# zitongbai/bipedal_control

Measured on AMD Instinct MI355X. Metric: MPC solves/s (H1, horizon=100), higher is better.
Workload: dtype f64; 1 GPU; Unitree H1 trot (template tiled from t = 0), horizon=100 intervals (dt 0.015), batch=256 per GPU perturbed initial states, cold start, 1 SQP iteration (BASELINE.json configs[1]); solver=sqp, global_batch=256, problems_on_rank0=256, shooting_nodes=108, nx=22, nu=22

## Files before the change

bipedal_control_amd/csrc/kernels/riccati_fast.h:

```cpp
#pragma once
#include <hip/hip_runtime.h>

#include "../device_model.h"
#include "riccati.h"
#include "project_node.h"
#include "linesearch.h"

namespace bpmpc {

struct RiccatiFastIO {
  RiccatiIO base;
  const double *Wt, *Qp, *Mt;
  const double* Vt;
  const double *lqA, *lqB, *lqb, *lqq, *lqr, *qrd, *gdt;
  const DeviceModel* model;
  const double* zero_one;
  const int* mode;
  double *Acl, *bcl;
  double *kff;
  double *mvec, *mscal;
  double* Kfull;
  double* prof;
  int k_lo, k_hi;
  double* carry;
  double reg;
  bool with_ls;
  ProblemLS ls;
};

__device__ __forceinline__ void lds_barrier() {
  __builtin_amdgcn_fence(__ATOMIC_RELEASE, "workgroup", "local");
  __builtin_amdgcn_s_barrier();
  __builtin_amdgcn_fence(__ATOMIC_ACQUIRE, "workgroup", "local");
}
__device__ __forceinline__ void lds_wave_sync() {
  __builtin_amdgcn_fence(__ATOMIC_RELEASE, "wavefront", "local");
  __builtin_amdgcn_wave_barrier();
  __builtin_amdgcn_fence(__ATOMIC_ACQUIRE, "wavefront", "local");
}
__device__ __forceinline__ double readlane_f64(double v, int lane) {
  const int lo = __builtin_amdgcn_readlane(__double2loint(v), lane);
  const int hi = __builtin_amdgcn_readlane(__double2hiint(v), lane);
  return __hiloint2double(hi, lo);
}
template <int NJ>
__device__ __forceinline__ void linesearch_begin_wave(double* partial , const ProblemLS& p, int lane) {
  constexpr int NX = 12 + NJ;
  {
    double a = 0.0, b = 0.0, c = 0.0;
    for (int k = lane; k < p.n_nodes; k += kWave) { a += p.node_perf[3 * k]; b += p.node_perf[3 * k + 1]; c += p.node_perf[3 * k + 2]; }
    if (lane < NX) { const double d = p.x0[lane] - p.x[lane]; b += d * d; }
    partial[lane] = a; partial[kWave + lane] = b; partial[2 * kWave + lane] = c;
  }
  lds_wave_sync();
  if (lane < 3) {
    double s = 0.0;
    for (int i = 0; i < kWave; ++i) s += partial[lane * kWave + i];
// ... 336 lines not shown
```

bipedal_control_amd/csrc/kernels/riccati_mfma.h:

```cpp
#pragma once
#include <hip/hip_runtime.h>

#include "riccati_fast.h"


namespace bpmpc {

typedef double v4d __attribute__((ext_vector_type(4)));

template <int LD>
struct LdsRows {
  static constexpr int kCols = LD;
  __host__ __device__ static constexpr int ix(int row, int col) { return row * LD + col; }
  static constexpr int size(int rows) { return rows * LD; }
};
template <int NBC>
struct LdsSwz {
  static constexpr int kCols = 16 * NBC, PS = 32 * NBC + 2;
  __host__ __device__ static constexpr int ix(int row, int col) { return (row >> 1) * PS + ((col >> 4) << 5) + (((row ^ (col >> 4)) & 1) << 4) + (col & 15); }
  static constexpr int size(int rows) { return ((rows + 1) / 2) * PS; }
};

template <int NJ>
struct RiccatiMfmaWorkspace {
// ... 142 lines not shown
        jix[e] = (ok && col == row) ? 1.0 : 0.0; jiy[e] = (ok && col + 1 == row) ? 1.0 : 0.0;
        jbo[e] = (ok && col == NX) ? row : -1; jb[e] = 0.0;
      }
    }
#pragma unroll
    for (int e = 0; e < SW; ++e) { const int p = tp + e * NLD; const bool ok = p < NPW; wo[e] = ok ? LW::ix(p / HW, 2 * (p % HW)) : -1; wc[e] = 2 * (p % HW); }
#pragma unroll
    for (int e = 0; e < SQ; ++e) { const int p = tp + e * NLD; const bool ok = p < NPQ; qo[e] = ok ? LN::ix(p / HQU, 2 * (p % HQU)) : -1; }
#pragma unroll
    for (int e = 0; e < SM; ++e) { const int p = tp + e * NLD; const bool ok = p < NPM; mo[e] = ok ? LW::ix(p / HW, 2 * (p % HW)) : -1; mc[e] = 2 * (p % HW); mr[e] = p / HW; }
  }
  __device__ __forceinline__ void prefetch(int nt, int mode) {
    const int cend = 16 * ((BC + nt + 15) >> 4);
#pragma unroll
    for (int e = 0; e < SW; ++e) {
      if constexpr (AM) { if ((e + 1) * NLD <= NPW || wo[e] >= 0) { const double2 v = *(wc[e] < cend ? gW + e * NLD : reinterpret_cast<const double2*>(pw.zero_one + 2)); wx[e] = v.x; wy[e] = v.y; } }
      else if (((e + 1) * NLD <= NPW || wo[e] >= 0) && wc[e] < cend) { const double2 v = gW[e * NLD]; wx[e] = v.x; wy[e] = v.y; }
    }
#pragma unroll
    for (int e = 0; e < SQ; ++e) if ((e + 1) * NLD <= NPQ || qo[e] >= 0) { const int p = tl + e * NLD; const double2 v = gQ[(p / HQU) * HQ + p % HQU]; qx[e] = v.x; qy[e] = v.y; }
#pragma unroll
    for (int e = 0; e < SM; ++e) {
      if constexpr (AM) { if ((e + 1) * NLD <= NPM || mo[e] >= 0) { const double2 v = *((mr[e] < nt && mc[e] < cend) ? gM + e * NLD : reinterpret_cast<const double2*>(pw.zero_one + 2)); mx[e] = v.x; my[e] = v.y; } }
      else if (((e + 1) * NLD <= NPM || mo[e] >= 0) && mr[e] < nt && mc[e] < cend) { const double2 v = gM[e * NLD]; mx[e] = v.x; my[e] = v.y; }
    }
    pw.prefetch(nt, mode);
    if constexpr (JR) {
      dtk = *gDt;
#pragma unroll
      for (int e = 0; e < SVJ; ++e) jb[e] = *(jbo[e] >= 0 ? gB + jbo[e] : pw.zero_one);
      gB -= NX; gDt -= 1;
    }
    gW -= PL::W_SIZE / 2; gQ -= PL::Q_SIZE / 2; gM -= PL::M_SIZE / 2;
  }
  __device__ __forceinline__ void stage(double* W, double* PW, double* Qq, double* M, double* rvec, int nt) const {
    stage_wm(W, M, rvec, nt);
    stage_pq(PW, Qq);
  }
  __device__ __forceinline__ void stage_wm(double* Wf, double* Mf, double* rvec, int nt) const {
    const int cend = 16 * ((BC + nt + 15) >> 4);
#pragma unroll
    for (int e = 0; e < SW; ++e)
      if ((e + 1) * NLD <= NPW || wo[e] >= 0) {
        const bool in = AM || wc[e] < cend; double2 v; v.x = in ? wx[e] : 0.0; v.y = in ? wy[e] : 0.0; *reinterpret_cast<double2*>(Wf + wo[e]) = v;
      }
#pragma unroll
    for (int e = 0; e < SM; ++e)
      if ((e + 1) * NLD <= NPM || mo[e] >= 0) {
        const bool in = AM || (mr[e] < nt && mc[e] < cend);
        double2 v; v.x = in ? mx[e] : 0.0; v.y = in ? my[e] : 0.0;
        *reinterpret_cast<double2*>(Mf + mo[e]) = v;
        if (mc[e] == NX) rvec[mr[e]] = v.x;
      }
    if constexpr (JR) {
#pragma unroll
      for (int e = 0; e < SVJ; ++e)
        if ((e + 1) * NLD <= NJ * HW || pw.vo[e] >= 0) {
          double2 v; v.x = __builtin_fma(dtk, pw.vx[e], jix[e] + jb[e]); v.y = __builtin_fma(dtk, pw.vy[e], jiy[e]);
          *reinterpret_cast<double2*>(Wf + pw.vo[e]) = v;
        }
    }
  }
  __device__ __forceinline__ void stage_pq(double* PW, double* Qf) const {
#pragma unroll
    for (int e = 0; e < SQ; ++e)
      if ((e + 1) * NLD <= NPQ || qo[e] >= 0) { double2 v; v.x = qx[e]; v.y = qy[e]; *reinterpret_cast<double2*>(Qf + qo[e]) = v; }
// ... 714 lines not shown
```

bipedal_control_amd/csrc/kernels/riccati_mfma8.h:

```cpp
#pragma once
#include <hip/hip_runtime.h>

#include "riccati_mfma.h"

namespace bpmpc {

typedef unsigned int bp8_u32x2 __attribute__((ext_vector_type(2)));
constexpr int kRiccati8Threads = 512;

template <int NJ>
struct RiccatiMfma8Workspace {
  static constexpr int NX = 12 + NJ, NU = 12 + NJ;
  static constexpr int RB = 32;
  static constexpr int RE = 16;
  static constexpr int WC = NX + 1 + NU;
  using LN = LdsSwz<2>;
  using LW = LdsSwz<(WC + 15) / 16>;
  static constexpr int ZN = 31;
  static_assert(NX + 1 <= 32 && NU <= 32, "two block rows / columns");
  alignas(16) double S[LN::size(RB)];
  alignas(16) double Qq[2][LN::size(RB)];
  alignas(16) double Sn[LN::size(RB)];
  alignas(16) double Zt[LN::size(RE)];
  alignas(16) double Yn[LN::size(RE)];
  alignas(16) double W[2][LW::size(RB)];
  alignas(16) double PW[2][LW::size(RB)];
  alignas(16) double SW[LW::size(RB)];
  alignas(16) double M[2][LW::size(RE)];
  alignas(16) double Mb[LW::size(RE)];
  double r[2][NU];
  int status;
  unsigned char nut[kMaxRiccatiStages];
  unsigned char mode[kMaxRiccatiStages];
};
template <class L>
__device__ __forceinline__ v4d sblk_load(const double* Mx, int r0, int c0, int l) {
  v4d c;
#pragma unroll
  for (int r = 0; r < 4; ++r) c[r] = lds1(Mx[L::ix(r0 + (l >> 4) + 4 * r, c0 + (l & 15))]);
  return c;
}
template <class L>
__device__ __forceinline__ void sblk_store(double* Mx, int r0, int c0, int l, v4d c) {
#pragma unroll
  for (int r = 0; r < 4; ++r) Mx[L::ix(r0 + (l >> 4) + 4 * r, c0 + (l & 15))] = c[r];
}

template <int ROWS, class Emit>
__device__ __forceinline__ bool forward_eliminate_wave(double (&v)[ROWS], int nt, Emit&& emit) {
  bool ok = true;
#pragma unroll
  for (int p = 0; p < ROWS; ++p) {
    if (p < nt) {
      double f[ROWS];
#pragma unroll
      for (int i = p; i < ROWS; ++i) f[i] = readlane_f64(v[i], p);
      ok = ok && (f[p] > 0.0);
      const double row = v[p] * fast_reciprocal(f[p]);
      emit(p, v[p], row);
#pragma unroll
      for (int i = p + 1; i < ROWS; ++i) v[i] -= f[i] * row;
      v[p] = row;
    }
  }
  return ok;
}
// ... 30 lines not shown
  const int k_top = (io.k_hi < N ? io.k_hi : N) - 1;
  const bool resumed = io.k_hi < N;
  {
    double* z = &ws.S[0];
    constexpr int total = (int)(offsetof(WS, status) / sizeof(double));
    for (int idx = tid; idx < total; idx += NT) z[idx] = 0.0;
  }
  __syncthreads();
  if (tid == 0) ws.status = resumed ? (int)io.carry[NXX + NX] : 0;
  if (!resumed && io.reg != 0.0 && tid < NX) ws.S[LN::ix(tid, tid)] = io.reg;
  if (resumed) {
    for (int idx = tid; idx < NXX; idx += NT) ws.S[LN::ix(idx / NX, idx % NX)] = io.carry[idx];
    if (tid < NX) ws.S[LN::ix(tid, NX)] = io.carry[NXX + tid];
  }
  int too_wide = 0;
  for (int idx = tid; idx < N && idx < kMaxRiccatiStages; idx += NT) {
    const int n = io.base.nut[idx];
    ws.nut[idx] = (unsigned char)n;
    ws.mode[idx] = (unsigned char)(n > 0 ? (io.mode[idx] & 3) : kModeEvent);
    too_wide |= n > RE ? 1 : 0;
  }
  if (__syncthreads_or(too_wide)) {
    if (tid == 0) {
      if (io.k_lo > 0) io.carry[NXX + NX] = 1.0;
      else { io.base.summary[0] = 0.0; io.base.summary[1] = 0.0; io.base.summary[2] = 0.0; io.base.summary[3] = 1.0; }
    }
    if (io.k_lo == 0 && io.with_ls && tid < kWave) linesearch_begin_wave<NJ>(&ws.S[0], io.ls, tid);
    return;
  }

  constexpr int NLD = kLoaders * kWave;
  PackedStageLoader<NJ, NLD, RE, LW::kCols, LN::kCols, true, !JW, LW, LN> ld;
  ld.init(io, (w - 4) * kWave + l, role_l, (size_t)(k_top > 0 ? k_top : 0));
  if (role_l && k_top >= io.k_lo) {
    const int kt = k_top > 0 ? k_top : 0, n0 = io.base.nut[kt];
    ld.prefetch(n0, n0 > 0 ? (io.mode[kt] & 3) : kModeEvent);
  }
  __syncthreads();
#ifdef BPMPC_RICCATI_PROFILE
  long long tacc[8] = {0, 0, 0, 0, 0, 0, 0, 0};
  long long tprev = clock64();
#define RM8PROF(slot) do { const long long tn_ = clock64(); tacc[slot] += tn_ - tprev; tprev = tn_; } while (0)
#define RM8OWN(phase) do { if (BPMPC_RICCATI_PROFILE == 10 + (phase)) tacc[7] += clock64() - tprev; } while (0)
#else
#define RM8PROF(slot) ((void)0)
#define RM8OWN(phase) ((void)0)
#endif

  constexpr int PSN = LN::PS, PSW = LW::PS;
  const int hk = lk >> 1, pk = lk & 1, hl = li >> 1, pl = li & 1;
  auto opaque = [](int v) { asm volatile("" : "+v"(v)); return v; };
  const int nP2a = opaque(hk * PSN + 16 * pk + li), nP2b = opaque(hk * PSN + 16 * (pk ^ 1) + li);
  const int wP2a = opaque(hk * PSW + 16 * pk + li), wP2b = opaque(hk * PSW + 16 * (pk ^ 1) + li);
  const int nP1a = opaque(hl * PSN + 16 * pl + lk), nP1b = opaque(hl * PSN + 16 * (pl ^ 1) + lk);
  const int nSV = opaque(hk * PSN + 16 * (pk ^ 1) + 32 + (NX & 15));
  static_assert(NX >= 16 && NX < 32, "column nx lies in block column 1");
  int wBC;
  { const int c = BC + li, cb = c >> 4; wBC = opaque(hk * PSW + 32 * cb + 16 * ((pk ^ cb) & 1) + (c & 15)); }
  int foW, foY, foB[4], snN, snP, wA3, suN, suZ, suY;
  {
    const int bw = w < 3 ? w : 3, r0 = 16 * (bw >> 1), c0 = 16 * (bw & 1);
    foW = opaque((r0 / 2) * PSW + 2 * c0 + ((bw & 1) ? wP2b : wP2a));
    foY = opaque(2 * c0 + ((bw & 1) ? wP2b : wP2a));
#pragma unroll
    for (int ks = 0; ks < 4; ++ks) foB[ks] = opaque(LW::ix(r0 + li, BC + 4 * ks + lk));
    const int sid = w & 1;
    snN = opaque(32 * sid + (sid ? nP2b : nP2a));
    snP = opaque(32 * sid + (sid ? wP2b : wP2a));
    const int ac3 = 16 + li < NX ? 16 + li : NX - 1;
// ... 30 lines not shown
    for (int r = 0; r < 4; ++r) { acl[r] = lds1(W[foW + 2 * r * PSW]); kf[r] = lds1(PW[foW + 2 * r * PSW]); }
    double ab[4], ap[4], yb[4];
#pragma unroll
    for (int ks = 0; ks < 4; ++ks) {
      yb[ks] = lds1(M[foY + 2 * ks * PSW]);
      ab[ks] = lds1(W[foB[ks]]);
      ap[ks] = lds1(PW[foB[ks]]);
    }
    __builtin_amdgcn_sched_barrier(0);
#pragma unroll
    for (int ks = 0; ks < 4; ++ks) {
      if (ks < ksn) {
        acl = __builtin_amdgcn_mfma_f64_16x16x4f64(ab[ks], yb[ks], acl, 0, 0, 0);
        kf = __builtin_amdgcn_mfma_f64_16x16x4f64(ap[ks], yb[ks], kf, 0, 0, 0);
      }
    }
    const unsigned ku = (unsigned)__builtin_amdgcn_readfirstlane(k);
    const unsigned sm = ku * (unsigned)(NXX * 8), sv = ku * (unsigned)(NX * 8);
#pragma unroll
    for (int r = 0; r < 4; ++r) {
      bp8_u32x2 va, vk;
      va.x = (unsigned)__double2loint(acl[r]); va.y = (unsigned)__double2hiint(acl[r]);
      vk.x = (unsigned)__double2loint(kf[r]); vk.y = (unsigned)__double2hiint(kf[r]);
      __builtin_amdgcn_raw_buffer_store_b64(va, rAcl, oom[r], sm, 0);
      __builtin_amdgcn_raw_buffer_store_b64(vk, rKf, oom[r], sm, 0);
      if (c0 != 0) {
        __builtin_amdgcn_raw_buffer_store_b64(va, rbcl, oov[r], sv, 0);
        __builtin_amdgcn_raw_buffer_store_b64(vk, rkff, oov[r], sv, 0);
      }
    }
  };

  auto finish_m = [&](int k, int buf) {
    if (l <= NX) {
      const int fm0 = 32 * (l >> 4) + 16 * ((l >> 4) & 1) + (l & 15);
      double yv[RE], rv[RE];
#pragma unroll
      for (int i = 0; i < RE; ++i) { yv[i] = ws.M[buf][(i >> 1) * PSW + ((i & 1) ? (fm0 ^ 16) : fm0)]; rv[i] = ws.r[buf][i]; }
      double m0 = l < NX ? ws.Qq[buf][LN::ix(l, NX)] : 0.0, m1 = 0.0;
#pragma unroll
      for (int i = 0; i < RE; i += 2) { m0 += yv[i] * rv[i]; m1 += yv[i + 1] * rv[i + 1]; }
      if (l < NX) io.mvec[(size_t)k * NX + l] = m0 + m1; else io.mscal[k] = m0 + m1;
    }
  };

  int pend_k = -1, pend_nt = 0;
  for (int k = k_top; k >= io.k_lo; --k) {
    const int nt = ws.nut[k];
    const int cur = k & 1;
    double* const W = ws.W[cur];
    double* const PW = ws.PW[cur];
    double* const Qq = ws.Qq[cur];
    double* const M = ws.M[cur];
    double* const rvec = ws.r[cur];
    const int ksn = (nt + 3) >> 2;
    const int nbc = (BC + nt + 15) >> 4;
    auto sn_block = [&](auto top_c) {
      constexpr bool TOP = decltype(top_c)::value;
      const int nb = TOP ? snN : 8 * PSN + 32 + nP2b;
      const int wa = TOP ? wP2a : wA3;
      const int wb = TOP ? snP : 32 + wP2b;
      v4d acc;
#pragma unroll
      for (int r = 0; r < 4; ++r) acc[r] = lds1(Qq[nb + 2 * r * PSN]);
      double a[KS], b[KS];
#pragma unroll
      for (int ks = 0; ks < KS; ++ks) {
        a[ks] = lds1(W[wa + 2 * ks * PSW]);
        b[ks] = lds1(ws.SW[wb + 2 * ks * PSW]);
      }
      if constexpr (!TOP) {
#pragma unroll
        for (int ks = 0; ks < KS; ++ks) a[ks] *= amask3;
      }
      __builtin_amdgcn_sched_barrier(0);
#pragma unroll
      for (int ks = 0; ks < KS; ++ks) acc = __builtin_amdgcn_mfma_f64_16x16x4f64(a[ks], b[ks], acc, 0, 0, 0);
#pragma unroll
      for (int r = 0; r < 4; ++r) ws.Sn[nb + 2 * r * PSN] = acc[r];
    };
    if (role_l) ld.stage(W, PW, Qq, M, rvec, nt);
    RM8OWN(0);
    lds_barrier();
    RM8PROF(0);
    if (role_l && k > io.k_lo) ld.prefetch(ws.nut[k - 1], ws.mode[k - 1]);
    if (w != 4 && w != 5) {
      const int id = w < 4 ? w : w - 2;
      if (id < 2 * nbc) {
        const int bi = id >= nbc ? 1 : 0;
        const int r0 = 16 * bi, c0 = 16 * (id - bi * nbc);
        const int row = r0 + li;
        const double half = row < NX ? 0.5 : 0.0;
        constexpr int KG1 = KS - 4;
        const int odd = (c0 >> 4) & 1;
        const int wb = 2 * c0 + (odd ? wP2b : wP2a);
        const int sx0 = 8 * bi * PSN + nP1a, sx1 = 8 * bi * PSN + 32 + nP1b;
        const int sy = 32 * bi + (bi ? nP2b : nP2a);
        double a[KS], b[KS], sv[4], ga[4];
#pragma unroll
        for (int ks = 0; ks < KS; ++ks) {
          const bool up = (bi == 0 && ks >= 4), lo = (bi != 0 && ks < 4);
          const int ex = (ks < 4 ? sx0 : sx1) + 4 * (ks & 3), ey = sy + 2 * ks * PSN;
          a[ks] = half * (lds1(ws.S[lo ? ey : ex]) + lds1(ws.S[up ? ex : ey]));
          b[ks] = lds1(W[wb + 2 * ks * PSW]);
        }
        const double smask = (c0 + li == NX) ? 1.0 : 0.0;
#pragma unroll
        for (int r = 0; r < 4; ++r) sv[r] = smask * lds1(ws.S[nSV + (8 * bi + 2 * r) * PSN]);
#pragma unroll
        for (int ks = 0; ks < 4; ++ks) ga[ks] = (bi == 0 || ks < KG1) ? lds1(W[wBC + (8 * bi + 2 * ks) * PSW]) : 0.0;
        v4d g;
#pragma unroll
        for (int r = 0; r < 4; ++r) g[r] = lds1(M[wb + 2 * r * PSW]);
        if (bi != 0) g = v4d{0.0, 0.0, 0.0, 0.0};
        __builtin_amdgcn_sched_barrier(0);
        v4d acc = {sv[0], sv[1], sv[2], sv[3]};
#pragma unroll
        for (int ks = 0; ks < KS; ++ks) acc = __builtin_amdgcn_mfma_f64_16x16x4f64(a[ks], b[ks], acc, 0, 0, 0);
// ... 62 lines not shown
        else BP_GJ_CASE(10, (forward_eliminate_rows<10, true>), back_substitute_rows)
      } else {
        if (nt <= 12) BP_GJ_CASE(12, forward_eliminate_wave<12>, back_substitute_wave)
        else BP_GJ_CASE(RE, forward_eliminate_wave<RE>, back_substitute_wave)
      }
#undef BP_GJ_CASE
#undef BP_EM
    } else {
      if (w == 4 || w == 5) sn_block(std::true_type{});
      if (w == 4) sn_block(std::false_type{});
      if (w == 5 && pend_k >= 0) finish_m(pend_k, cur ^ 1);
      if ((w < 3 || role_f) && pend_k >= 0) finish_outputs(pend_k, cur ^ 1, pend_nt, w < 3 ? w : 3);
      RM8PROF(6);
      lds_barrier();
      RM8PROF(3);
      if (role_c && w != 2) {
        v4d acc;
#pragma unroll
        for (int r = 0; r < 4; ++r) acc[r] = lds1(ws.Sn[suN + 2 * r * PSN]);
        double ag[4], yb[4];
#pragma unroll
        for (int ks = 0; ks < 4; ++ks) {
          ag[ks] = -lds1(ws.Zt[suZ + 2 * ks * PSN]);
          yb[ks] = lds1(ws.Yn[suY + 2 * ks * PSN]);
        }
        __builtin_amdgcn_sched_barrier(0);
#pragma unroll
        for (int ks = 0; ks < 4; ++ks)
          if (ks < ksn) acc = __builtin_amdgcn_mfma_f64_16x16x4f64(ag[ks], yb[ks], acc, 0, 0, 0);
#pragma unroll
        for (int r = 0; r < 4; ++r) ws.S[suN + 2 * r * PSN] = acc[r];
      }
    }
    pend_k = k; pend_nt = nt;
    RM8OWN(4);
    RM8PROF(4);
  }
#ifdef BPMPC_RICCATI_PROFILE
#if BPMPC_RICCATI_PROFILE == 2
  if (io.prof && l == 0) io.prof[w] = (double)tacc[6];
#elif BPMPC_RICCATI_PROFILE >= 10
  if (io.prof && l == 0) io.prof[w] = (double)tacc[7];
#else
  if (io.prof && tid == 0)
    for (int i = 0; i < 5; ++i) io.prof[i] = (double)tacc[i];
  if (io.prof && tid == 7 * kWave) io.prof[7] = (double)tacc[6];
#endif
#endif
  __syncthreads();
  if ((w < 3 || role_f) && pend_k >= 0) finish_outputs(pend_k, pend_k & 1, pend_nt, w < 3 ? w : 3);
  if (w == 5 && pend_k >= 0) finish_m(pend_k, pend_k & 1);
  __syncthreads();
  if (io.k_lo > 0) {
    for (int idx = tid; idx < NXX; idx += NT) { const int r = idx / NX, c = idx % NX; io.carry[idx] = (r >= 16 && c < 16) ? ws.S[LN::ix(c, r)] : ws.S[LN::ix(r, c)]; }
    if (tid < NX) io.carry[NXX + tid] = ws.S[LN::ix(tid, NX)];
    if (tid == 0) io.carry[NXX + NX] = (double)ws.status;
    return;
  }
  {
    const int st = ws.status;
    __syncthreads();
#ifdef BPMPC_RICCATI_PROFILE
    const long long tr0 = clock64();
#endif
    constexpr int kRingChunk = 4;
    using RR = RolloutRing<NJ, NT, kRingChunk>;
    constexpr int kRingCap = RR::cap((int)(offsetof(WS, status) / sizeof(double)));
    static_assert(kRingCap >= 128, "roll-out history");
    riccati_rollout_ring<NJ, NT, kRingChunk>(reinterpret_cast<double*>(&ws), kRingCap, st, io);
#ifdef BPMPC_RICCATI_PROFILE
    if (BPMPC_RICCATI_PROFILE == 1 && io.prof && tid == 0) io.prof[5] = (double)(clock64() - tr0);
#endif
  }
}

}
```

bipedal_control_amd/csrc/launch.h:

```cpp
#pragma once
#include <hip/hip_runtime.h>

#include <cstddef>

#include "device_model.h"
#include "kernels/linesearch.h"
#include "kernels/node_lq.h"
#include "kernels/project_node.h"
#include "kernels/riccati_fast.h"
#include "kernels/linearize_fast.h"

namespace bpmpc {

struct Buffers {
  int *g_kind, *g_mode, *g_nodes;
  double *g_dt, *g_start, *g_zref, *g_zdref;
  int* p_grid;
  double *p_x0, *p_tgt_t, *p_tgt_x;
  int* p_tgt_n;
  double *x, *u, *x_init, *u_init, *xref;
  double *A, *B, *b, *Q, *R, *P, *q, *r, *c, *C, *D, *e, *perf;
  int* nc;
  double *Px, *Pu, *Pe, *At, *Bt, *bt, *Qt, *Rt, *Pt, *qt, *rt;
  double *Wt, *Qp, *Mt;
// ... 14 lines not shown
  int *rg_gait, *rg_status, *rg_rows, *lib_i;
  double* ric_carry;
  double* zero_page;
  double *trial_perf, *base, *alpha, *stats;
  int *done, *active, *iterations, *remaining;
};

struct DdpBuffers {
  int cap;
  int nv;
  double alpha_v[kMaxDdpSteps];
  double* lff;
  double *rec_t, *rec_x, *rec_u, *cost;
  int* rec_n;
  double *end_x, *end_u;
  int *roll_steps, *roll_status;
  double *sol_t, *sol_x, *sol_u;
  int* sol_n;
  double *merit0, *merit, *alpha, *update_is;
  int *accepted, *failed, *n_points;
};

constexpr int kLinMaxEvents = 8;
struct Launch {
  const DeviceModel* model;
  Buffers buf;
  int batch, N;
  int k0, klen;
  int cold;
  int feedback;
  int serial_legs;
  LineSearchSettings ls;
  double reg_prim;
  int lin_ev_n, lin_inter;
  int lin_ev[kLinMaxEvents];
  int ilqr;
  double ilqr_shift;
};


template <int NJ>
__device__ __forceinline__ NodeInputs node_inputs(const Launch& L, int b, int k) {
  constexpr int NX = 12 + NJ, NU = 12 + NJ;
  const int g = L.buf.p_grid[b];
  const size_t gs = (size_t)g * L.N + k, s = (size_t)b * L.N + k;
  NodeInputs in;
  in.kind = L.buf.g_kind[gs];
  in.mode = L.buf.g_mode[gs];
  in.dt = L.buf.g_dt[gs];
  in.x = L.buf.x + ((size_t)b * (L.N + 1) + k) * NX;
  in.xnext = in.x + NX;
  in.u = L.buf.u + s * NU;
  in.xref = L.buf.xref + s * NX;
  in.zref = L.buf.g_zref + gs * 4;
  in.zdref = L.buf.g_zdref + gs * 4;
  return in;
}

template <int NJ>
__device__ __forceinline__ NodeInputs node_inputs_on_grid(const Launch& L, int b, int k, int g) {
  constexpr int NX = 12 + NJ, NU = 12 + NJ;
  const size_t gs = (size_t)g * L.N + k, s = (size_t)b * L.N + k;
  NodeInputs in;
  in.kind = L.buf.g_kind[gs];
  in.mode = L.buf.g_mode[gs];
  in.dt = L.buf.g_dt[gs];
// ... 41 lines not shown
    if (io.with_ls && tid_ < kWave) linesearch_begin_wave<NJ>(lds_scratch, io.ls, tid_);
    return false;
  }
  const size_t s0 = (size_t)b * L.N;
  double* dx0 = L.buf.dx0 + (size_t)b * NX;
  if (tid_ < NX) dx0[tid_] = L.buf.p_x0[(size_t)b * NX + tid_] - L.buf.x[(size_t)b * (L.N + 1) * NX + tid_];
  __syncthreads();
  io.base.N = L.buf.g_nodes[L.buf.p_grid[b]];
  io.base.nut = L.buf.nut + s0;
  io.base.At = L.buf.At + s0 * NX * NX; io.base.Bt = L.buf.Bt + s0 * NX * NU; io.base.bt = L.buf.bt + s0 * NX;
  io.base.Qt = L.buf.Qt + s0 * NX * NX; io.base.Rt = L.buf.Rt + s0 * NU * NU; io.base.Pt = L.buf.Pt + s0 * NU * NX;
  io.base.qt = L.buf.qt + s0 * NX; io.base.rt = L.buf.rt + s0 * NU;
  io.Wt = L.buf.Wt + s0 * PackedLq<NJ>::W_SIZE; io.Qp = L.buf.Qp + s0 * PackedLq<NJ>::Q_SIZE; io.Mt = L.buf.Mt + s0 * PackedLq<NJ>::M_SIZE;
  io.base.Px = L.buf.Px + s0 * NU * NX; io.base.Pu = L.buf.Pu + s0 * NU * NU; io.base.Pe = L.buf.Pe + s0 * NU;
  io.Vt = L.buf.Vt + s0 * NJ * PackedLq<NJ>::WP;
  io.mode = L.buf.g_mode + (size_t)L.buf.p_grid[b] * L.N;
  io.zero_one = L.buf.zero_page;
  io.lqA = L.buf.A + s0 * NX * NX; io.lqB = L.buf.B + s0 * NX * NU; io.lqb = L.buf.b + s0 * NX; io.lqq = L.buf.q + s0 * NX; io.lqr = L.buf.r + s0 * NU;
  io.qrd = L.buf.qrd + s0 * kQrdStride; io.gdt = L.buf.g_dt + (size_t)L.buf.p_grid[b] * L.N;
  io.model = L.model;
  io.base.dx0 = dx0;
  io.base.Kt = nullptr; io.base.kt = nullptr;
  io.base.dx = L.buf.dx + (size_t)b * (L.N + 1) * NX; io.base.du = L.buf.du + s0 * NU;
  io.base.K = nullptr;
  io.base.summary = L.buf.summary + (size_t)b * 4;
  io.Acl = L.buf.Acl + s0 * NX * NX; io.bcl = L.buf.bcl + s0 * NX; io.kff = L.buf.kff + s0 * NU;
  io.mvec = L.buf.mvec + s0 * NX; io.mscal = L.buf.mscal + s0;
  io.Kfull = L.buf.K + s0 * NU * NX;
  io.prof = L.buf.rprof ? L.buf.rprof + (size_t)b * 8 : nullptr;
  io.k_lo = L.k0;
  io.k_hi = L.k0 + L.klen;
  io.carry = L.buf.ric_carry + (size_t)b * (NX * NX + NX + 2);
  io.reg = L.reg_prim;
  return true;
}

}
```

bipedal_control_amd/csrc/solver.h:

```cpp
#pragma once
#include <hip/hip_runtime.h>

#include <algorithm>
#include <cstring>
#include <map>
#include <string>
#include <utility>
#include <vector>

#include "../../include/bpmpc.h"
#include "device_handle.h"
#include "kernel_launchers.h"
#include "launch.h"
#include "kernels/reference_device.h"

namespace bpmpc {

struct KernelTimer {
  std::vector<std::pair<hipEvent_t, hipEvent_t>> pending;
  double total_ms = 0.0;
  int launches = 0;
};

}
// ... 12 lines not shown
    if (demand > cap) {
      if (base) (void)hipHostFree(base);
      base = nullptr; cap = 0;
      const size_t want = std::max<size_t>(2 * demand, size_t(1) << 20);
      if (hipHostMalloc(reinterpret_cast<void**>(&base), want) == hipSuccess) cap = want; else base = nullptr;
    }
    used = 0; demand = 0;
  }
  void* take(size_t bytes) {
    const size_t at = (used + 63) & ~size_t(63);
    demand = ((demand + 63) & ~size_t(63)) + bytes;
    if (!base || at + bytes > cap) return nullptr;
    used = at + bytes;
    return base + at;
  }
  void release() { if (base) (void)hipHostFree(base); base = nullptr; cap = used = demand = 0; }
};

struct bpmpc_solver {
  HostStaging staging;
  PinnedArena pin_up, pin_down;
  char* xfer = nullptr;
  size_t xfer_cap = 0;
  RobotModel rm;
  DeviceModel dm;
  DeviceModel* d_model = nullptr;
  bpmpc_settings settings{};
  int nx = 0, nu = 0;
  int batch = 0, n_grids = 0, n_nodes_max = 0;
  int num_cus = 256;
  bool structured_project = false;
  int riccati_wave = 1;
  bool lin_compact = true;
  bool force_tables = false;
  bool wt_joint_rows = false;
  bool sweep_wave_regime() const { return riccati_wave == 2 || riccati_wave == 4 || ((riccati_wave == 1 || riccati_wave == 3) && batch > 2 * num_cus); }
  bool sweep_two_per_simd() const { return sweep_wave_regime() && (riccati_wave >= 3 || (riccati_wave == 1 && batch > 4 * num_cus)); }
  bool sweep_completes_joint_rows() const { return !wt_joint_rows && structured_project && !settings.reference_kernels; }
  int r8_rounds = 0;
  int eight_wave_rounds() const { return r8_rounds > 0 ? r8_rounds : (rm.nj == 10 ? 3 : 1); }
  bool sweep_eight_waves() const { return riccati_wave != 2 && riccati_wave != 4 && batch <= eight_wave_rounds() * num_cus; }
  bool has_solution = false;
  bool has_rollout = false;
  bool rollout_unchecked = false;
  double* tick_x = nullptr;
  bool loop_from_tick = false;
  int* restart_flag = nullptr;
  int* restart_mask = nullptr;
  double* restart_x = nullptr;
  bool restart_pending = false, restart_wait = false;
  std::vector<int> grid_kind;
  int max_rows = kMaxEqRows;
  int max_vel_rows = 12;
  bool cold = true;
  hipStream_t stream = nullptr;
  bool own_stream = false;
  hipStream_t producer_stream = nullptr;
  hipEvent_t ev_go = nullptr;
  std::vector<hipEvent_t> ev_chunk;
  Buffers buf{};
  std::vector<void*> allocations;
  std::map<std::string, std::pair<void*, size_t>> named;
  std::map<std::string, bool> is_int;
  std::vector<double> node_times;
  std::vector<int> grid_nodes, grid_of_problem;
  std::map<std::string, KernelTimer> timers;
  int* h_remaining = nullptr;
  LineSearchSettings ls{};

  template <typename T>
  T* alloc(const char* name, size_t count, bool integer = false) {
    void* p = nullptr;
    HIP_CHECK(hipMalloc(&p, count * sizeof(T)));
    HIP_CHECK(hipMemsetAsync(p, 0, count * sizeof(T), stream));
    allocations.push_back(p);
    if (name) { named[name] = {p, count}; is_int[name] = integer; }
    return static_cast<T*>(p);
  }

  Launch launch_params() const {
    Launch L;
    L.model = d_model;
    L.buf = buf;
    L.batch = batch;
    L.N = settings.max_nodes;
    L.k0 = 0;
    L.klen = n_nodes_max > 0 ? n_nodes_max : settings.max_nodes;
    L.cold = cold ? 1 : 0;
    L.serial_legs = (dm.serial_legs && !force_tables) ? 1 : 0;
    L.feedback = feedback();
    L.ls = ls;
    L.reg_prim = settings.reg_prim;
    L.lin_ev_n = -1; L.lin_inter = 0;
    for (int i = 0; i < kLinMaxEvents; ++i) L.lin_ev[i] = 0;
    if (n_grids == 1 && lin_compact && !grid_kind.empty() && (int)grid_nodes.size() == 1) {
      const int n = grid_nodes[0];
      int ne = 0;
      for (int k = 0; k < n; ++k)
        if (grid_kind[k] == 1) { if (ne < kLinMaxEvents) L.lin_ev[ne] = k; ++ne; }
      if (ne <= kLinMaxEvents && n == L.klen) { L.lin_ev_n = ne; L.lin_inter = n - ne; }
    }
    L.ilqr = is_ddp() ? 1 : 0;
    L.ilqr_shift = is_ddp() ? rm.ddp.ls_hessian_correction_multiple : 0.0;
    return L;
  }

  static constexpr unsigned kTimingEventFlags = hipEventDisableSystemFence;
  bool timed(const char* cls) const { return settings.profile == 1 || (settings.profile == 2 && std::strcmp(cls, "linearize") == 0); }
  void time_begin(const char* cls, hipEvent_t* a, hipEvent_t* b, hipStream_t on = nullptr) {
    if (!timed(cls)) return;
    HIP_CHECK(hipEventCreateWithFlags(a, kTimingEventFlags));
    if (hipEventCreateWithFlags(b, kTimingEventFlags) != hipSuccess) { (void)hipEventDestroy(*a); throw DeviceError("hipEventCreate failed"); }
    if (hipEventRecord(*a, on ? on : stream) != hipSuccess) { (void)hipEventDestroy(*a); (void)hipEventDestroy(*b); throw DeviceError("hipEventRecord failed"); }
  }
  void time_end(const char* cls, hipEvent_t a, hipEvent_t b, hipStream_t on = nullptr) {
    if (!timed(cls)) return;
    HIP_CHECK(hipEventRecord(b, on ? on : stream));
    KernelTimer& t = timers[cls];
    t.pending.emplace_back(a, b);
    if (t.pending.size() > 4096) collect_timers();
  }
  void launch_linearize_fast(hipStream_t on, const Launch& L, int nodes) {
    if (!timed("linearize")) { kl::linearize_fast(nj(), settings.materialize_lq != 0, nodes, on, L); return; }
    hipEvent_t a, b;
    HIP_CHECK(hipEventCreateWithFlags(&a, kTimingEventFlags));
// ... 99 lines not shown
```

bipedal_control_amd/csrc/solver.hip:

```cpp
#include <hip/hip_runtime.h>

#include <cmath>
#include <cstdint>
#include <algorithm>
#include <cstring>
#include <map>
#include <tuple>
#include <memory>
#include <stdexcept>
#include <string>
#include <vector>

#include "solver.h"
#include "reference_gen.h"
#include "kernels/rollout.h"

#define TIMED_ON(on, cls, ...)                                                      \
  do {                                                                              \
    hipEvent_t ev_a_, ev_b_;                                                        \
    time_begin(cls, &ev_a_, &ev_b_, on);                                            \
    __VA_ARGS__;                                                                    \
    time_end(cls, ev_a_, ev_b_, on);                                                \
    HIP_CHECK(hipGetLastError());                                                   \
  } while (0)
// ... 755 lines not shown
  }
  std::unique_ptr<bpmpc_solver> s(new bpmpc_solver);
  const int rc = guarded(BPMPC_ERR_IO, [&]() -> int {
    s->rm = model_of(model);
    if (s->rm.nj != 10 && s->rm.nj != 12) { set_last_error("only 10- and 12-joint bipeds are instantiated"); return BPMPC_ERR_UNSUPPORTED; }
    if (settings->reg_prim != 0.0 && settings->reference_kernels) { set_last_error("reg_prim is implemented by the fast kernels only"); return BPMPC_ERR_UNSUPPORTED; }
    if (!(settings->reg_prim >= 0.0)) { set_last_error("reg_prim must be >= 0"); return BPMPC_ERR_INVALID_ARGUMENT; }
    s->dm = make_device_model(s->rm);
    s->settings = *settings;
    if (settings->solver != BPMPC_SOLVER_SQP && settings->solver != BPMPC_SOLVER_DDP) { set_last_error("bpmpc_solver_create: unknown solver"); return BPMPC_ERR_INVALID_ARGUMENT; }
    if (settings->feedback_policy < 0 || settings->feedback_policy > 2) { set_last_error("bpmpc_solver_create: feedback_policy must be 0, 1 or 2"); return BPMPC_ERR_INVALID_ARGUMENT; }
    if (settings->solver == BPMPC_SOLVER_DDP) {
      const DdpConfig& d = s->rm.ddp;
      if (d.algorithm != 1) { set_last_error("DDP: only ddp.algorithm ILQR is implemented (SLQ integrates continuous-time Riccati equations)"); return BPMPC_ERR_UNSUPPORTED; }
      if (d.strategy != 0) { set_last_error("DDP: only ddp.strategy LINE_SEARCH is implemented"); return BPMPC_ERR_UNSUPPORTED; }
      if (d.ls_hessian_correction_strategy != 0) { set_last_error("DDP: only lineSearch.hessianCorrectionStrategy DIAGONAL_SHIFT is implemented"); return BPMPC_ERR_UNSUPPORTED; }
      if (d.max_num_iterations != 1 || settings->sqp_iterations > 1) { set_last_error("DDP: one ILQR iteration per run (ddp.maxNumIterations 1): later iterations live on the roll-out's adaptive time grid"); return BPMPC_ERR_UNSUPPORTED; }
      if (!(d.ls_min_step_length > 0.0) || !(d.ls_max_step_length >= d.ls_min_step_length)) { set_last_error("DDP: lineSearch.minStepLength / maxStepLength"); return BPMPC_ERR_INVALID_ARGUMENT; }
      if (ddp_step_lengths(d, kMaxDdpSteps - 1) > kMaxDdpSteps - 1) {
        set_last_error("DDP: lineSearch.minStepLength / maxStepLength ask for more than " + std::to_string(kMaxDdpSteps - 1) + " step lengths (contraction rate 0.5), the line search table holds no more");
        return BPMPC_ERR_UNSUPPORTED;
      }
      if (d.use_feedback_policy && settings->feedback_policy != 2) { set_last_error("DDP: ddp.useFeedbackPolicy true is not implemented (the gains live on the nominal grid, the solution on the roll-out's time points)"); return BPMPC_ERR_UNSUPPORTED; }
      if (settings->feedback_policy == 1) { set_last_error("DDP: feedback_policy 1 (LinearController) is not implemented for the DDP solution"); return BPMPC_ERR_UNSUPPORTED; }
      s->settings.return_gains = 1;
      s->settings.pipeline_chunks = 1;
    }
    s->nx = s->rm.nx; s->nu = s->rm.nu;
    HIP_CHECK(hipSetDevice(settings->device));
    { hipDeviceProp_t prop; HIP_CHECK(hipGetDeviceProperties(&prop, settings->device)); s->num_cus = prop.multiProcessorCount; }
    { const char* e = std::getenv("BPMPC_WT_JOINT_ROWS"); s->wt_joint_rows = e && e[0] == '1'; }
    { const char* e = std::getenv("BPMPC_LIN_TABLES"); s->force_tables = e && e[0] == '1'; }
    { const char* e = std::getenv("BPMPC_LIN_COMPACT"); s->lin_compact = !(e && e[0] == '0'); }
    { const char* e = std::getenv("BPMPC_RICCATI_WAVE"); s->riccati_wave = e ? std::atoi(e) : 1; }
    { const char* e = std::getenv("BPMPC_R8_ROUNDS"); s->r8_rounds = e ? std::atoi(e) : 0; }
    {
      bool block_diagonal = true;
      for (int c = 0; c < 12; ++c)
        for (int j = 12; j < s->nu; ++j) block_diagonal = block_diagonal && s->dm.R[c * s->nu + j] == 0.0 && s->dm.R[j * s->nu + c] == 0.0;
      const char* e = std::getenv("BPMPC_DENSE_PROJECT");
      s->structured_project = block_diagonal && !(e && e[0] == '1');
    }
    if (s->is_ddp() && !(s->dm.serial_legs && !s->force_tables)) s->settings.reference_kernels = 1;
    if (settings->stream) { s->stream = static_cast<hipStream_t>(settings->stream); }
    else { HIP_CHECK(hipStreamCreateWithFlags(&s->stream, hipStreamNonBlocking)); s->own_stream = true; }
    if (s->settings.pipeline_chunks <= 0) s->settings.pipeline_chunks = 1;
    if (s->settings.pipeline_chunks > 16) s->settings.pipeline_chunks = 16;
    HIP_CHECK(hipStreamCreateWithFlags(&s->producer_stream, hipStreamNonBlocking));
    HIP_CHECK(hipEventCreateWithFlags(&s->ev_go, hipEventDisableTiming));
    s->ev_chunk.resize(s->settings.pipeline_chunks);
    for (auto& e : s->ev_chunk) HIP_CHECK(hipEventCreateWithFlags(&e, hipEventDisableTiming));
    {
      std::vector<char> host(kLinImageOffset + sizeof(LinFastShared<12, true>), 0);
      std::memcpy(host.data(), &s->dm, sizeof(DeviceModel));
      if (s->rm.nj == 10) fill_shared_image<10>(s->dm, *reinterpret_cast<LinFastShared<10, true>*>(host.data() + kLinImageOffset));
      else if (s->rm.nj == 12) fill_shared_image<12>(s->dm, *reinterpret_cast<LinFastShared<12, true>*>(host.data() + kLinImageOffset));
      HIP_CHECK(hipMalloc(reinterpret_cast<void**>(&s->d_model), host.size()));
      HIP_CHECK(hipMemcpy(s->d_model, host.data(), host.size(), hipMemcpyHostToDevice));
    }
    HIP_CHECK(hipHostMalloc(reinterpret_cast<void**>(&s->h_remaining), sizeof(int)));
    const SqpConfig& q = s->rm.sqp;
    s->ls = LineSearchSettings{q.g_max, q.g_min, q.alpha_decay, q.alpha_min, q.gamma_c, q.armijo_factor, q.delta_tol, q.cost_tol,
                               settings->sqp_iterations > 0 ? settings->sqp_iterations : q.sqp_iteration};
    allocate(s.get());
    HIP_CHECK(hipStreamSynchronize(s->stream));
    return BPMPC_OK;
// ... 202 lines not shown
```

Measured before the change: 343,200 solves/s.

## Add fast path for event stages in MFMA8 Riccati backward sweep

Event stages (no inputs, nt==0) in the 512-thread MFMA Riccati kernel now skip the full stage staging and factorisation. Only the jump offset vector is fetched, S is updated as a symmetrised identity-plus-offset product with one MFMA block per wave, and the trivial closed-loop outputs (identity Acl, zero gains) are written directly. The loader gains a skip() that advances its global pointers, and buffer parity now follows a toggled counter instead of k&1. This removes the wasted loads and compute for the few event nodes, at the cost of extra branching and a new path enabled by default behind an env flag.

```diff
diff --git a/bipedal_control_amd/csrc/kernels/riccati_fast.h b/bipedal_control_amd/csrc/kernels/riccati_fast.h
--- a/bipedal_control_amd/csrc/kernels/riccati_fast.h
+++ b/bipedal_control_amd/csrc/kernels/riccati_fast.h
@@ -23,6 +23,7 @@
   double* prof;
   int k_lo, k_hi;
   double* carry;
+  int event_fast;
   double reg;
   bool with_ls;
   ProblemLS ls;
diff --git a/bipedal_control_amd/csrc/kernels/riccati_mfma.h b/bipedal_control_amd/csrc/kernels/riccati_mfma.h
--- a/bipedal_control_amd/csrc/kernels/riccati_mfma.h
+++ b/bipedal_control_amd/csrc/kernels/riccati_mfma.h
@@ -198,6 +198,15 @@
       gB -= NX; gDt -= 1;
     }
     gW -= PL::W_SIZE / 2; gQ -= PL::Q_SIZE / 2; gM -= PL::M_SIZE / 2;
+  }
+  __device__ __forceinline__ double event_b(int row) const {
+    if (!JR || row < 12) return reinterpret_cast<const double*>(gW + (row * (HW - 1) + NX / 2))[0];
+    return gB[row];
+  }
+  __device__ __forceinline__ void skip() {
+    gW -= PL::W_SIZE / 2; gQ -= PL::Q_SIZE / 2; gM -= PL::M_SIZE / 2;
+    pw.gV -= (NJ * WP) / 2; pw.gPe -= NU;
+    if constexpr (JR) { gB -= NX; gDt -= 1; }
   }
   __device__ __forceinline__ void stage(double* W, double* PW, double* Qq, double* M, double* rvec, int nt) const {
     stage_wm(W, M, rvec, nt);
diff --git a/bipedal_control_amd/csrc/kernels/riccati_mfma8.h b/bipedal_control_amd/csrc/kernels/riccati_mfma8.h
--- a/bipedal_control_amd/csrc/kernels/riccati_mfma8.h
+++ b/bipedal_control_amd/csrc/kernels/riccati_mfma8.h
@@ -32,6 +32,7 @@
   int status;
   unsigned char nut[kMaxRiccatiStages];
   unsigned char mode[kMaxRiccatiStages];
+  alignas(16) double evb[32];
 };
 template <class L>
 __device__ __forceinline__ v4d sblk_load(const double* Mx, int r0, int c0, int l) {
@@ -128,9 +129,20 @@
   constexpr int NLD = kLoaders * kWave;
   PackedStageLoader<NJ, NLD, RE, LW::kCols, LN::kCols, true, !JW, LW, LN> ld;
   ld.init(io, (w - 4) * kWave + l, role_l, (size_t)(k_top > 0 ? k_top : 0));
+  const int evf = io.event_fast;
+  auto prefetch_stage = [&](int n, int mode) {
+    if (evf != 0 && __builtin_amdgcn_readfirstlane(n) == 0) {
+      int lv = l;
+      asm volatile("" : "+v"(lv));
+      if (w == 4 && lv < NX) ld.wx[0] = ld.event_b(lv);
+      ld.skip();
+    } else {
+      ld.prefetch(n, mode);
+    }
+  };
   if (role_l && k_top >= io.k_lo) {
     const int kt = k_top > 0 ? k_top : 0, n0 = io.base.nut[kt];
-    ld.prefetch(n0, n0 > 0 ? (io.mode[kt] & 3) : kModeEvent);
+    prefetch_stage(n0, n0 > 0 ? (io.mode[kt] & 3) : kModeEvent);
   }
   __syncthreads();
 #ifdef BPMPC_RICCATI_PROFILE
@@ -227,6 +239,8 @@
   };
 
   auto finish_m = [&](int k, int buf) {
+    int l = tid & 63;
+    asm volatile("" : "+v"(l));
     if (l <= NX) {
       const int fm0 = 32 * (l >> 4) + 16 * ((l >> 4) & 1) + (l & 15);
       double yv[RE], rv[RE];
@@ -240,9 +254,11 @@
   };
 
   int pend_k = -1, pend_nt = 0;
+  int cur = 0;
   for (int k = k_top; k >= io.k_lo; --k) {
     const int nt = ws.nut[k];
-    const int cur = k & 1;
+    const bool event = evf != 0 && __builtin_amdgcn_readfirstlane(nt) == 0;
+    int wsc = 0;
     double* const W = ws.W[cur];
     double* const PW = ws.PW[cur];
     double* const Qq = ws.Qq[cur];
@@ -274,11 +290,85 @@
 #pragma unroll
       for (int r = 0; r < 4; ++r) ws.Sn[nb + 2 * r * PSN] = acc[r];
     };
-    if (role_l) ld.stage(W, PW, Qq, M, rvec, nt);
+    if (!event) {
+      if (role_l) ld.stage(W, PW, Qq, M, rvec, nt);
+    } else {
+      int wv = w;
+      asm volatile("" : "+v"(wv));
+      wsc = __builtin_amdgcn_readfirstlane(wv);
+      if (wsc == 4) {
+        int lv = l;
+        asm volatile("" : "+v"(lv));
+        if (lv < 4 * KS) ws.evb[lv] = lv < NX ? ((!JW && lv >= 12) ? 0.0 + ld.wx[0] : ld.wx[0]) : 0.0;
+      }
+    }
     RM8OWN(0);
     lds_barrier();
     RM8PROF(0);
-    if (role_l && k > io.k_lo) ld.prefetch(ws.nut[k - 1], ws.mode[k - 1]);
+    if (role_l && k > io.k_lo) prefetch_stage(ws.nut[k - 1], ws.mode[k - 1]);
+    if (event) {
+      v4d acc = {0.0, 0.0, 0.0, 0.0};
+      auto s_block = [&](auto bi_c, auto bc_c) {
+        constexpr int bi = decltype(bi_c)::value, bc = decltype(bc_c)::value, c0 = 16 * bc;
+        int lv = l;
+        asm volatile("" : "+v"(lv));
+        const int li = lv & 15, lk = lv >> 4;
+        const int row = 16 * bi + li, col = c0 + li;
+        const double half = row < NX ? 0.5 : 0.0;
+        const int sx0 = 8 * bi * PSN + nP1a, sx1 = 8 * bi * PSN + 32 + nP1b;
+        const int sy = 32 * bi + (bi ? nP2b : nP2a);
+        double a[KS], b[KS], sv[4];
+#pragma unroll
+        for (int ks = 0; ks < KS; ++ks) {
+          const bool up = (bi == 0 && ks >= 4), lo = (bi != 0 && ks < 4);
+          const int ex = (ks < 4 ? sx0 : sx1) + 4 * (ks & 3), ey = sy + 2 * ks * PSN;
+          a[ks] = half * (lds1(ws.S[lo ? ey : ex]) + lds1(ws.S[up ? ex : ey]));
+          const int kk = 4 * ks + lk;
+          if constexpr (bc == 0) b[ks] = (kk == col) ? 1.0 : 0.0;
+          else { const double bk = lds1(ws.evb[kk]); b[ks] = col == NX ? bk : ((kk == col && kk < NX) ? 1.0 : 0.0); }
+        }
+        const double smask = (col == NX) ? 1.0 : 0.0;
+#pragma unroll
+        for (int r = 0; r < 4; ++r) sv[r] = smask * lds1(ws.S[nSV + (8 * bi + 2 * r) * PSN]);
+        __builtin_amdgcn_sched_barrier(0);
+        acc = v4d{sv[0], sv[1], sv[2], sv[3]};
+#pragma unroll
+        for (int ks = 0; ks < KS; ++ks) acc = __builtin_amdgcn_mfma_f64_16x16x4f64(a[ks], b[ks], acc, 0, 0, 0);
+#pragma unroll
+        for (int r = 0; r < 4; ++r) {
+          const int rr = 16 * bi + lk + 4 * r;
+          acc[r] = ((rr == col && rr < NX) ? io.reg : 0.0) + acc[r];
+        }
+      };
+      if (wsc == 0) s_block(std::integral_constant<int, 0>{}, std::integral_constant<int, 0>{});
+      else if (wsc == 1) s_block(std::integral_constant<int, 0>{}, std::integral_constant<int, 1>{});
+      else if (wsc == 3) s_block(std::integral_constant<int, 1>{}, std::integral_constant<int, 1>{});
+      else if (wsc == 2 || wsc >= 6) {
+        int lv = l;
+        asm volatile("" : "+v"(lv));
+        const int t = (wsc == 2 ? 0 : wsc - 5) * kWave + lv;
+        const unsigned ku = (unsigned)__builtin_amdgcn_readfirstlane(k);
+        const unsigned sm = ku * (unsigned)(NXX * 8), sv = ku * (unsigned)(NX * 8);
+        auto b64 = [](double v) { bp8_u32x2 r; r.x = (unsigned)__double2loint(v); r.y = (unsigned)__double2hiint(v); return r; };
+        for (int idx = t; idx < NXX; idx += 3 * kWave) {
+          __builtin_amdgcn_raw_buffer_store_b64(b64((idx / NX == idx % NX) ? 1.0 : 0.0), rAcl, (unsigned)idx * 8u, sm, 0);
+          __builtin_amdgcn_raw_buffer_store_b64(b64(0.0), rKf, (unsigned)idx * 8u, sm, 0);
+        }
+        if (t < NX) {
+          __builtin_amdgcn_raw_buffer_store_b64(b64(ws.evb[t]), rbcl, (unsigned)t * 8u, sv, 0);
+          __builtin_amdgcn_raw_buffer_store_b64(b64(0.0), rkff, (unsigned)t * 8u, sv, 0);
+          io.mvec[(size_t)k * NX + t] = 0.0;
+        }
+        if (t == NX) io.mscal[k] = 0.0;
+      }
+      lds_barrier();
+      if (wsc == 0 || wsc == 1 || wsc == 3) {
+#pragma unroll
+        for (int r = 0; r < 4; ++r) ws.S[suN + 2 * r * PSN] = acc[r];
+      }
+      RM8PROF(5);
+      continue;
+    }
     if (w != 4 && w != 5) {
       const int id = w < 4 ? w : w - 2;
       if (id < 2 * nbc) {
@@ -407,7 +497,7 @@
         for (int r = 0; r < 4; ++r) ws.S[suN + 2 * r * PSN] = acc[r];
       }
     }
-    pend_k = k; pend_nt = nt;
+    pend_k = k; pend_nt = nt; cur ^= 1;
     RM8OWN(4);
     RM8PROF(4);
   }
@@ -423,8 +513,12 @@
 #endif
 #endif
   __syncthreads();
-  if ((w < 3 || role_f) && pend_k >= 0) finish_outputs(pend_k, pend_k & 1, pend_nt, w < 3 ? w : 3);
-  if (w == 5 && pend_k >= 0) finish_m(pend_k, pend_k & 1);
+  {
+    const int wq = opaque(w), bw = wq < 3 ? wq : 3;
+    foY = 32 * (bw & 1) + ((bw & 1) ? wP2b : wP2a);
+  }
+  if ((w < 3 || role_f) && pend_k >= 0) finish_outputs(pend_k, cur ^ 1, pend_nt, w < 3 ? w : 3);
+  if (w == 5 && pend_k >= 0) finish_m(pend_k, cur ^ 1);
   __syncthreads();
   if (io.k_lo > 0) {
     for (int idx = tid; idx < NXX; idx += NT) { const int r = idx / NX, c = idx % NX; io.carry[idx] = (r >= 16 && c < 16) ? ws.S[LN::ix(c, r)] : ws.S[LN::ix(r, c)]; }
diff --git a/bipedal_control_amd/csrc/launch.h b/bipedal_control_amd/csrc/launch.h
--- a/bipedal_control_amd/csrc/launch.h
+++ b/bipedal_control_amd/csrc/launch.h
@@ -70,6 +70,7 @@
   int serial_legs;
   LineSearchSettings ls;
   double reg_prim;
+  int ric_event_fast;
   int lin_ev_n, lin_inter;
   int lin_ev[kLinMaxEvents];
   int ilqr;
@@ -177,6 +178,7 @@
   io.k_hi = L.k0 + L.klen;
   io.carry = L.buf.ric_carry + (size_t)b * (NX * NX + NX + 2);
   io.reg = L.reg_prim;
+  io.event_fast = L.ric_event_fast;
   return true;
 }
 
diff --git a/bipedal_control_amd/csrc/solver.h b/bipedal_control_amd/csrc/solver.h
--- a/bipedal_control_amd/csrc/solver.h
+++ b/bipedal_control_amd/csrc/solver.h
@@ -68,6 +68,7 @@
   bool structured_project = false;
   int riccati_wave = 1;
   bool lin_compact = true;
+  int ric_event_fast = 1;
   bool force_tables = false;
   bool wt_joint_rows = false;
   bool sweep_wave_regime() const { return riccati_wave == 2 || riccati_wave == 4 || ((riccati_wave == 1 || riccati_wave == 3) && batch > 2 * num_cus); }
@@ -127,6 +128,7 @@
     L.feedback = feedback();
     L.ls = ls;
     L.reg_prim = settings.reg_prim;
+    L.ric_event_fast = ric_event_fast;
     L.lin_ev_n = -1; L.lin_inter = 0;
     for (int i = 0; i < kLinMaxEvents; ++i) L.lin_ev[i] = 0;
     if (n_grids == 1 && lin_compact && !grid_kind.empty() && (int)grid_nodes.size() == 1) {
diff --git a/bipedal_control_amd/csrc/solver.hip b/bipedal_control_amd/csrc/solver.hip
--- a/bipedal_control_amd/csrc/solver.hip
+++ b/bipedal_control_amd/csrc/solver.hip
@@ -811,6 +811,7 @@
     { const char* e = std::getenv("BPMPC_WT_JOINT_ROWS"); s->wt_joint_rows = e && e[0] == '1'; }
     { const char* e = std::getenv("BPMPC_LIN_TABLES"); s->force_tables = e && e[0] == '1'; }
     { const char* e = std::getenv("BPMPC_LIN_COMPACT"); s->lin_compact = !(e && e[0] == '0'); }
+    { const char* e = std::getenv("BPMPC_RICCATI_EVENT_FAST"); s->ric_event_fast = e ? (e[0] == '0' ? 0 : (e[0] == '2' ? 2 : 1)) : 1; }
     { const char* e = std::getenv("BPMPC_RICCATI_WAVE"); s->riccati_wave = e ? std::atoi(e) : 1; }
     { const char* e = std::getenv("BPMPC_R8_ROUNDS"); s->r8_rounds = e ? std::atoi(e) : 0; }
     {
```

Measured after the change: 339,700 solves/s. -1.0%, worse.
